# 87003697/DynamiCrafter

Measured on AMD Instinct MI355X. Metric: frames/sec (and denoising-step ms), 16f@576x1024, DDIM 50, higher is better.
Workload: dtype bf16; 1 GPU; inference_1024_v1.0.yaml: 1 clip/GPU, 16 frames, latent 72x128, DDIM 50 uniform_trailing eta=1, CFG 7.5 batched (cond+uncond), guidance_rescale 0.7, v-param+ZTSNR+dynamic rescale, hipGraph-captured step; clips_per_gpu=1, parallelism=dp1 over 1 distinct clips (no data-path collective), conditioning=local (1 rank), outputs_finite=True

## Files before the change

### dynamicrafter_amd/_hip.py

```python
import ctypes as C
import os
import threading

_HERE = os.path.dirname(os.path.abspath(__file__))
LIB_PATH = os.environ.get("DC_HIP_LIB") or os.path.join(_HERE, "csrc", "libdcrafter_hip.so")

DC_GEMM_OUT_F32 = 1
DC_GEMM_GEGLU = 2
DC_GEMM_GELU = 4


class DcGemmParams(C.Structure):
    _fields_ = [
        ("A", C.c_void_p), ("W", C.c_void_p), ("C", C.c_void_p), ("bias", C.c_void_p),
        ("rowvec", C.c_void_p), ("residual", C.c_void_p),
        ("lda", C.c_int), ("ldc", C.c_int), ("ldr", C.c_int), ("rowvec_ld", C.c_int),
        ("rows_per_vec", C.c_int),
        ("M", C.c_int), ("N", C.c_int), ("K", C.c_int), ("n_pad", C.c_int),
        ("mode", C.c_int), ("Cin", C.c_int),
        ("IH", C.c_int), ("IW", C.c_int), ("OH", C.c_int), ("OW", C.c_int),
        ("stride", C.c_int), ("pad", C.c_int), ("ups", C.c_int),
        ("T", C.c_int), ("HW", C.c_int),
        ("flags", C.c_int), ("alpha", C.c_float),
        ("workspace", C.c_void_p), ("workspace_bytes", C.c_longlong),
    ]


class DcDdimParams(C.Structure):
    _fields_ = [
        ("a_t", C.c_void_p), ("a_prev", C.c_void_p), ("sigma_t", C.c_void_p), ("sqrt_one_minus_at", C.c_void_p),
        ("sqrt_acp_t", C.c_void_p), ("sqrt_1macp_t", C.c_void_p), ("scale_ratio", C.c_void_p),
        ("step_index", C.c_void_p),
        ("index", C.c_int), ("v_param", C.c_int),
        ("cfg_scale", C.c_float), ("cfg_img", C.c_float), ("guidance_rescale", C.c_float),
        ("temperature", C.c_float),
        ("e_nchw", C.c_int), ("noise_step_stride", C.c_int64),
    ]


class DcDpmParams(C.Structure):
    _fields_ = [
        ("A", C.c_void_p), ("alpha_t", C.c_void_p), ("alpha_p_r", C.c_void_p), ("k", C.c_void_p), ("N", C.c_void_p),
        ("sqrt_one_minus_at", C.c_void_p), ("sqrt_acp_t", C.c_void_p), ("sqrt_1macp_t", C.c_void_p),
        ("scale_ratio", C.c_void_p), ("step_index", C.c_void_p),
        ("index", C.c_int), ("v_param", C.c_int),
        ("cfg_scale", C.c_float), ("cfg_img", C.c_float), ("guidance_rescale", C.c_float),
        ("temperature", C.c_float),
        ("e_nchw", C.c_int), ("noise_step_stride", C.c_int64), ("x0_hist", C.c_void_p),
    ]


class DcSdsParams(C.Structure):
    _fields_ = [
        ("c1", C.c_void_p), ("c2", C.c_void_p), ("w", C.c_void_p), ("step_size", C.c_void_p), ("bc2_sqrt", C.c_void_p),
        ("step_index", C.c_void_p), ("index", C.c_int), ("weight_type", C.c_int), ("x0_param", C.c_int),
        ("e_nchw", C.c_int), ("cfg_scale", C.c_float), ("guidance_rescale", C.c_float),
        ("beta2", C.c_float), ("eps", C.c_float), ("one_minus_beta1", C.c_float), ("one_minus_beta2", C.c_float),
        ("decay", C.c_float), ("grad_scale", C.c_float), ("noise_step_stride", C.c_int64), ("loss", C.c_void_p),
    ]


_P, _I, _F, _L = C.c_void_p, C.c_int, C.c_float, C.c_int64
SIGNATURES = {
    "dc_gemm_conv": (_I, [C.POINTER(DcGemmParams), _P]),
    "dc_gemm_workspace_bytes": (_L, []),
    "dc_gemm_last_variant": (C.c_char_p, []),
    "dc_gemm_set_plan": (_I, [_I]),
    "dc_groupnorm": (_I, [_P, _I, _P, _I, _P, _P, _I, _I, _I, _I, _F, _I, _P, _P]),
    "dc_groupnorm_workspace_bytes": (_L, [_I, _I, _I]),
    "dc_layernorm": (_I, [_P, _I, _P, _I, _P, _P, _I, _I, _F, _P]),
    "dc_flash_attn_d64": (_I, [_P, _P, _P, _P, _I, _I, _I, _I, _I, _I, _I, _I, _L, _L, _F, _I, _F, _P]),
    "dc_ff_geglu_fused320": (_I, [_P, _I, _P, _P, _F, _P, _P, _P, _P, _P, _I, _P, _I, _I, _P]),
    "dc_ff_geglu_proj_fused320": (_I, [_P, _I, _P, _P, _F, _P, _P, _P, _P, _P, _P, _P, _I, _P, _I, _I, _P]),
    "dc_ln_linear": (_I, [_P, _I, _I, _P, _P, _F, _P, _P, _P, _I, _I, _I, _P]),
    "dc_ln_qkv_temporal_attn320": (_I, [_P, _I, _P, _P, _F, _P, _P, _I, _I, _I, _I, _F, _P]),
    "dc_ln_qkv_temporal_attn640": (_I, [_P, _I, _P, _P, _F, _P, _P, _I, _I, _I, _I, _F, _P]),
    "dc_gn_silu_tconv3": (_I, [_P, _I, _I, _P, _P, _P, _I, _P, _P, _P, _I, _P, _I, _I, _I, _I, _I, _P]),
    "dc_groupnorm_stats": (_I, [_P, _I, _I, _I, _I, _I, _F, _P, _P, _P]),
    "dc_gn_linear": (_I, [_P, _I, _I, _P, _P, _P, _I, _I, _P, _P, _P, _I, _I, _I, _P]),
    "dc_flash_attn_set_mode": (_I, [_I, _F]),
    "dc_linear_residual": (_I, [_P, _I, _I, _P, _P, _P, _I, _P, _I, _I, _I, _P]),
    "dc_cross_attn_dual_d64": (_I, [_P, _P, _P, _P, _P, _P, _I, _I, _I, _I, _I, _I, _I, _I, _L, _L, _F, _F, _P]),
    "dc_temporal_attn_d64": (_I, [_P, _I, _P, _I, _I, _I, _I, _I, _F, _P]),
    "dc_gemv_small": (_I, [_P, _I, _P, _P, _P, _I, _I, _I, _I, _I, _I, _I, _P]),
    "dc_timestep_embedding": (_I, [_P, _P, _I, _P, _I, _I, _F, _P]),
    "dc_pack_latent": (_I, [_P, _P, _P, _I, _I, _I, _I, _I, _I, _I, _P]),
    "dc_pack_latent_windows": (_I, [_P, _P, _P, _P, _P] + [_I] * 13 + [_P]),
    "dc_window_merge": (_I, [_P, _I, _P, _I, _P, _P, _P] + [_I] * 12 + [_P]),
    "dc_nchw_to_rows": (_I, [_P, _P, _I, _I, _I, _I, _F, _P]),
    "dc_rows_to_nchw": (_I, [_P, _I, _I, _P, _I, _I, _I, _F, _P]),
    "dc_im2col3x3_c8": (_I, [_P, _I, _P, _I, _I, _I, _I, _P]),
    "dc_copy2d": (_I, [_P, _I, _P, _I, _I, _I, _P]),
    "dc_build_context": (_I, [_P, _P, _I, _I, _I, _I, _I, _P]),
    "dc_softmax_rows": (_I, [_P, _I, _P, _I, _I, _I, _P]),
    "dc_transpose": (_I, [_P, _I, _P, _I, _I, _I, _P]),
    "dc_add_rows": (_I, [_P, _I, _P, _I, _P, _I, _I, _I, _P]),
    "dc_vae_sample": (_I, [_P, _I, _P, _P, _I, _I, _I, _F, _P]),
    "dc_ddim_step": (_I, [C.POINTER(DcDdimParams), _P, _P, _P, _I, _P, _P, _P, _P, _I, _I, _I, _P, _P]),
    "dc_dpmpp_step": (_I, [C.POINTER(DcDpmParams), _P, _P, _P, _I, _P, _P, _P, _P, _I, _I, _I, _P, _P]),
    "dc_sds_noise": (_I, [C.POINTER(DcSdsParams), _P, _P, _P, _I, _L, _P]),
    "dc_sds_step": (_I, [C.POINTER(DcSdsParams), _P, _P, _I, _P, _P, _P, _P, _I, _I, _I, _P, _P]),
    "dc_attn_small": (_I, [_P, _P, _P, _P, _I, _I, _I, _I, _I, _I, _I, _I, _I, _F, _I, _P]),
    "dc_attn_small_lds_bytes": (_L, [_I, _I]),
    "dc_clip_preprocess": (_I, [_P, _P, _P, _P, _I, _I, _I, _I, _I, _I, _I, C.POINTER(_F), C.POINTER(_F), _P]),
    "dc_patchify": (_I, [_P, _P, _I, _I, _I, _I, _I, _I, _P]),
    "dc_embed_tokens": (_I, [_P, _P, _P, _P, _I, _I, _I, _I, _P]),
    "dc_frames_to_u8": (_I, [_P, _P, _I, _I, _I, _I, _I, _P]),
    "dc_jpeg_dct_quant": (_I, [_P, _P, _P, _I, _I, _I, _P]),
    "dc_jpeg_entropy": (_I, [_P, _P, _P, _I, _I, _I, _I, _L, _P]),
    "dc_jpeg_pack": (_I, [_P, _P, _P, _P, _P, _I, _I, _L, _L, _P]),
    "dc_mask_blend": (_I, [_P, _P, _P, _P, _P, _P, _P, _I, _L, _L, _I, _P]),
    "dc_advance_counter": (_I, [_P, _P]),
    "dc_stream_create": (_I, [C.POINTER(_P)]),
    "dc_stream_destroy": (_I, [_P]),
    "dc_stream_sync": (_I, [_P]),
    "dc_graph_begin_capture": (_I, [_P]),
    "dc_graph_end_capture": (_I, [_P, C.POINTER(_P)]),
    "dc_graph_launch": (_I, [_P, _P]),
    "dc_graph_destroy": (_I, [_P]),
    "dc_event_create": (_I, [C.POINTER(_P)]),
    "dc_event_record": (_I, [_P, _P]),
    "dc_event_elapsed_ms": (_I, [_P, _P, C.POINTER(_F)]),
    "dc_event_destroy": (_I, [_P]),
    "dc_error_word_read": (_I, [C.POINTER(C.c_int), _I]),
    "dc_version": (C.c_char_p, []),
}

_lib = None
_lock = threading.Lock()


def lib():
    global _lib
    if _lib is not None:
        return _lib
    with _lock:
        if _lib is None:
            if not os.path.exists(LIB_PATH):
                raise RuntimeError(
                    f"{LIB_PATH} not found: build it with dynamicrafter_amd/csrc/build.sh "
                    "(or __graft_entry__.build()); the HIP extension is mandatory, there is no fallback")
            import torch
            l = C.CDLL(LIB_PATH)
            for name, (res, args) in SIGNATURES.items():
                fn = getattr(l, name)
                fn.restype = res
                fn.argtypes = args
            _lib = l
    return _lib


ERROR_WORD_BITS = {1: "gemm_pipe320x16_kernel: LDS counter wait timed out",
                   2: "flash_attn_d64_pipe_kernel: K/V ring counter wait timed out",
                   4: "gemm_pp_kernel: LDS counter wait timed out"}


def check_error_word(what="", reset=True):
    w = C.c_int(0)
    check(lib().dc_error_word_read(C.byref(w), 1 if reset else 0), "dc_error_word_read")
    if w.value:
        names = [v for k, v in ERROR_WORD_BITS.items() if w.value & k] or [f"unknown bits {w.value:#x}"]
        raise RuntimeError(f"HIP kernels reported a failed wait ({what or 'error word'} = {w.value:#x}): " + "; ".join(names)
                           + " - results since the last check are NOT valid")


def check(code, what):
    if code != 0:
        raise RuntimeError(f"{what} failed with code {code}"
                           + (" (DC_ERR_SHAPE)" if code == -1 else " (DC_ERR_ARG)" if code == -2 else " (hipError_t)"))
```

### dynamicrafter_amd/csrc/norms.hip

```cpp
#include "dc_common.h"
#include "dcrafter_hip.h"
#include <stdlib.h>

namespace {

struct GnGeom { int chunks; int rows_per_chunk; };

__host__ __device__ inline GnGeom gn_geom(int n_inst, int rows_per_inst) {
    int chunks = (2048 + n_inst - 1) / n_inst;
    int rpc = (rows_per_inst + chunks - 1) / chunks;
    if (rpc < 64) rpc = 64;
    GnGeom g;
    g.rows_per_chunk = rpc;
    g.chunks = (rows_per_inst + rpc - 1) / rpc;
    return g;
}

__global__ void gn_partial_kernel(const bf16_t* __restrict__ x, int ldx, int C, int groups, int rows_per_inst,
                                  int rows_per_chunk, int chunks, int vecs, int rpp, float2* __restrict__ partial) {
    extern __shared__ float sm[];
    const int inst = blockIdx.y, chunk = blockIdx.x;
    const int v = threadIdx.x % vecs;
    const int ro = threadIdx.x / vecs;
    const int r_begin = chunk * rows_per_chunk;
// ... 43 lines not shown
        for (int rr = 0; rr < rpp; ++rr) {
            const int first = r_begin + rr;
            const float nb = first < r_end ? (float)((r_end - first + rpp - 1) / rpp) : 0.f;
            if (nb == 0.f) continue;
            for (int c = 0; c < cpg; ++c) {
                const float mb = sm_s[rr * C + g * cpg + c], qb = sm_q[rr * C + g * cpg + c];
                const float nn = n + nb;
                const float w = nb * __builtin_amdgcn_rcpf(nn);
                const float delta = mb - mean;
                mean += delta * w;
                m2 += qb + delta * delta * (n * w);
                n = nn;
            }
        }
        partial[((size_t)inst * chunks + chunk) * groups + g] = make_float2(mean, m2);
    }
}

__global__ __launch_bounds__(64) void gn_finalize_kernel(const float2* __restrict__ partial, int chunks, int groups,
                                                         int rows_per_inst, int rows_per_chunk, int cpg, float eps,
                                                         float2* __restrict__ stats) {
    const int g = blockIdx.x, inst = blockIdx.y;
    float n = 0.f, mean = 0.f, m2 = 0.f;
    for (int c = threadIdx.x; c < chunks; c += 64) {
        const float2 p = partial[((size_t)inst * chunks + c) * groups + g];
        int rows = rows_per_inst - c * rows_per_chunk;
        if (rows > rows_per_chunk) rows = rows_per_chunk;
        const float nb = (float)rows * (float)cpg;
        const float nn = n + nb;
        const float w = nb * __builtin_amdgcn_rcpf(nn);
        const float delta = p.x - mean;
        mean += delta * w;
        m2 += p.y + delta * delta * (n * w);
        n = nn;
    }
#pragma unroll
    for (int o = 32; o > 0; o >>= 1) {
        const float nb = __shfl_xor(n, o, 64), mb = __shfl_xor(mean, o, 64), qb = __shfl_xor(m2, o, 64);
        const float nn = n + nb;
        if (nn > 0.f) {
            const float w = nb * __builtin_amdgcn_rcpf(nn);
            const float delta = mb - mean;
            mean += delta * w;
            m2 += qb + delta * delta * (n * w);
            n = nn;
        }
    }
    if (threadIdx.x == 0) {
        float var = m2 / n;
        if (var < 0.f) var = 0.f;
        stats[(size_t)inst * groups + g] = make_float2(mean, rsqrtf(var + eps));
    }
}

template <bool FIN>
__global__ void gn_apply_kernel(const bf16_t* __restrict__ x, int ldx, bf16_t* __restrict__ y, int ldy,
                                const float* __restrict__ gamma, const float* __restrict__ beta, int C, int groups,
                                int rows_per_inst, int rows_per_chunk, int vecs, int rpp, int silu,
                                const float2* __restrict__ stats, int chunks, float eps) {
    const int inst = blockIdx.y, chunk = blockIdx.x;
    __shared__ float2 st_s[64];
    if constexpr (FIN) {
        const int t = threadIdx.x, sub = t & 7;
        const int gpp = (int)blockDim.x >> 3;
        const float cpg = (float)(C / groups);
        for (int g0 = 0; g0 < groups; g0 += gpp) {
            const int g = g0 + (t >> 3);
            float n = 0.f, mean = 0.f, m2 = 0.f;
            if (g < groups) {
                for (int c = sub; c < chunks; c += 8) {
                    const float2 p = stats[((size_t)inst * chunks + c) * groups + g];
                    int rows = rows_per_inst - c * rows_per_chunk;
                    if (rows > rows_per_chunk) rows = rows_per_chunk;
                    const float nb = (float)rows * cpg;
                    const float nn = n + nb;
                    const float w = nb * __builtin_amdgcn_rcpf(nn);
                    const float delta = p.x - mean;
                    mean += delta * w;
                    m2 += p.y + delta * delta * (n * w);
                    n = nn;
                }
            }
#pragma unroll
            for (int o = 1; o < 8; o <<= 1) {
                const float nb = __shfl_xor(n, o, 64), mb = __shfl_xor(mean, o, 64), qb = __shfl_xor(m2, o, 64);
                const float nn = n + nb;
                if (nn > 0.f) {
                    const float lo_n = (sub & o) ? nb : n, lo_m = (sub & o) ? mb : mean, lo_q = (sub & o) ? qb : m2;
                    const float hi_n = (sub & o) ? n : nb, hi_m = (sub & o) ? mean : mb, hi_q = (sub & o) ? m2 : qb;
                    const float w = hi_n * __builtin_amdgcn_rcpf(nn);
                    const float delta = hi_m - lo_m;
                    mean = lo_m + delta * w;
                    m2 = lo_q + hi_q + delta * delta * (lo_n * w);
                    n = nn;
                }
            }
            if (g < groups && sub == 0) {
                float var = m2 / n;
                if (var < 0.f) var = 0.f;
                st_s[g] = make_float2(mean, rsqrtf(var + eps));
            }
        }
        __syncthreads();
    }
    const int v = threadIdx.x % vecs;
    const int ro = threadIdx.x / vecs;
    const int r_begin = chunk * rows_per_chunk;
    int r_end = r_begin + rows_per_chunk;
    if (r_end > rows_per_inst) r_end = rows_per_inst;
    const int cpg = C / groups;
    float sc[8], sh[8];
#pragma unroll
    for (int e = 0; e < 8; ++e) {
        const int c = v * 8 + e;
        const float2 st = FIN ? st_s[c / cpg] : stats[(size_t)inst * groups + c / cpg];
        const float g = gamma[c] * st.y;
        sc[e] = g;
        sh[e] = beta[c] - st.x * g;
    }
    const bf16_t* xb = x + (size_t)inst * rows_per_inst * ldx + v * 8;
    bf16_t* yb = y + (size_t)inst * rows_per_inst * ldy + v * 8;
    int r = r_begin + ro;
    for (; r + 7 * rpp < r_end; r += 8 * rpp) {
        uint4 raw[8];
#pragma unroll
        for (int u = 0; u < 8; ++u) raw[u] = *reinterpret_cast<const uint4*>(xb + (size_t)(r + u * rpp) * ldx);
#pragma unroll
        for (int u = 0; u < 8; ++u) {
            float f[8];
            unpack_bf8(raw[u], f);
#pragma unroll
            for (int e = 0; e < 8; ++e) {
                float t = f[e] * sc[e] + sh[e];
                if (silu) t = silu_f(t);
                f[e] = t;
            }
            *reinterpret_cast<uint4*>(yb + (size_t)(r + u * rpp) * ldy) = pack_bf8(f);
        }
    }
    for (; r < r_end; r += rpp) {
        const uint4 raw = *reinterpret_cast<const uint4*>(xb + (size_t)r * ldx);
        float f[8];
        unpack_bf8(raw, f);
#pragma unroll
        for (int e = 0; e < 8; ++e) {
            float t = f[e] * sc[e] + sh[e];
            if (silu) t = silu_f(t);
            f[e] = t;
        }
        *reinterpret_cast<uint4*>(yb + (size_t)r * ldy) = pack_bf8(f);
    }
}

template <int MAXV>
__global__ __launch_bounds__(256) void layernorm_kernel(const bf16_t* __restrict__ x, int ldx, bf16_t* __restrict__ y,
                                                        int ldy, const float* __restrict__ gamma,
                                                        const float* __restrict__ beta, int rows, int C, float eps) {
    const int lane = threadIdx.x & 63;
    const int wave = threadIdx.x >> 6;
    const int vecs = C >> 3;
    const float invC = 1.0f / (float)C;
    for (int row0 = (blockIdx.x * 4 + wave) * 2; row0 < rows; row0 += gridDim.x * 8) {
        float f[2][MAXV][8];
        float s[2] = {0.f, 0.f};
#pragma unroll
        for (int u = 0; u < 2; ++u) {
            const int row = row0 + u < rows ? row0 + u : rows - 1;
#pragma unroll
            for (int j = 0; j < MAXV; ++j) {
                const int v = lane + 64 * j;
                if (v < vecs) {
                    const uint4 raw = *reinterpret_cast<const uint4*>(x + (size_t)row * ldx + v * 8);
                    unpack_bf8(raw, f[u][j]);
#pragma unroll
                    for (int e = 0; e < 8; ++e) s[u] += f[u][j][e];
                }
            }
        }
#pragma unroll
        for (int u = 0; u < 2; ++u) {
            const int row = row0 + u;
            const float mean = wave_sum(s[u]) * invC;
            float q = 0.f;
#pragma unroll
            for (int j = 0; j < MAXV; ++j) {
                const int v = lane + 64 * j;
                if (v < vecs) {
#pragma unroll
                    for (int e = 0; e < 8; ++e) { const float d = f[u][j][e] - mean; q += d * d; }
                }
            }
            const float rstd = rsqrtf(wave_sum(q) * invC + eps);
            if (row < rows) {
#pragma unroll
                for (int j = 0; j < MAXV; ++j) {
                    const int v = lane + 64 * j;
                    if (v < vecs) {
                        float o[8];
#pragma unroll
                        for (int e = 0; e < 8; ++e) {
                            const int c = v * 8 + e;
                            o[e] = (f[u][j][e] - mean) * rstd * gamma[c] + beta[c];
                        }
                        *reinterpret_cast<uint4*>(y + (size_t)row * ldy + v * 8) = pack_bf8(o);
                    }
                }
            }
        }
    }
}

}

extern "C" int64_t dc_groupnorm_workspace_bytes(int n_inst, int groups, int rows_per_inst) {
    const GnGeom g = gn_geom(n_inst, rows_per_inst);
    return (int64_t)sizeof(float2) * ((int64_t)n_inst * g.chunks * groups + (int64_t)n_inst * groups) + 256;
}

extern "C" int dc_groupnorm(const uint16_t* x, int ldx, uint16_t* y, int ldy, const float* gamma, const float* beta,
                            int C, int groups, int n_inst, int rows_per_inst, float eps, int silu,
                            float* workspace, void* stream_) {
    hipStream_t stream = (hipStream_t)stream_;
    if (!x || !y || !gamma || !beta || !workspace) return DC_ERR_ARG;
    if (C % 8 != 0 || groups <= 0 || groups > 64 || C % groups != 0 || ldx % 8 != 0 || ldy % 8 != 0) return DC_ERR_SHAPE;
    if (n_inst <= 0 || rows_per_inst <= 0) return DC_ERR_SHAPE;
    const int vecs = C / 8;
    if (vecs > 1024) return DC_ERR_SHAPE;
    int rpp = 256 / vecs;
    if (rpp < 1) rpp = 1;
    const int threads = vecs * rpp;
    const GnGeom g = gn_geom(n_inst, rows_per_inst);
    float2* partial = reinterpret_cast<float2*>(workspace);
    float2* stats = partial + (size_t)n_inst * g.chunks * groups;
    const size_t lds = (size_t)2 * rpp * C * sizeof(float);
    if (lds > 64 * 1024) return DC_ERR_SHAPE;
    hipLaunchKernelGGL(gn_partial_kernel, dim3(g.chunks, n_inst), dim3(threads), lds, stream, x, ldx, C, groups,
                       rows_per_inst, g.rows_per_chunk, g.chunks, vecs, rpp, partial);
    DC_CHECK_LAUNCH();
    static const bool fuse_fin = [] { const char* e = getenv("DC_GN_FUSE_FINALIZE"); return !(e && e[0] == '0'); }();
    if (fuse_fin && g.chunks <= 64 && threads % 8 == 0) {
        hipLaunchKernelGGL(gn_apply_kernel<true>, dim3(g.chunks, n_inst), dim3(threads), 0, stream, x, ldx, y, ldy, gamma, beta,
                           C, groups, rows_per_inst, g.rows_per_chunk, vecs, rpp, silu, (const float2*)partial, g.chunks, eps);
        DC_CHECK_LAUNCH();
        return 0;
    }
    hipLaunchKernelGGL(gn_finalize_kernel, dim3(groups, n_inst), dim3(64), 0, stream, partial, g.chunks, groups, rows_per_inst,
                       g.rows_per_chunk, C / groups, eps, stats);
    DC_CHECK_LAUNCH();
    hipLaunchKernelGGL(gn_apply_kernel<false>, dim3(g.chunks, n_inst), dim3(threads), 0, stream, x, ldx, y, ldy, gamma, beta,
                       C, groups, rows_per_inst, g.rows_per_chunk, vecs, rpp, silu, (const float2*)stats, g.chunks, eps);
    DC_CHECK_LAUNCH();
    return 0;
}

extern "C" int dc_groupnorm_stats(const uint16_t* x, int ldx, int C, int groups, int n_inst, int rows_per_inst, float eps,
                                  float* workspace, float* stats_out, void* stream_) {
    hipStream_t stream = (hipStream_t)stream_;
    if (!x || !workspace || !stats_out) return DC_ERR_ARG;
    if (C % 8 != 0 || groups <= 0 || groups > 64 || C % groups != 0 || ldx % 8 != 0) return DC_ERR_SHAPE;
    if (n_inst <= 0 || rows_per_inst <= 0) return DC_ERR_SHAPE;
    const int vecs = C / 8;
    if (vecs > 1024) return DC_ERR_SHAPE;
    int rpp = 256 / vecs;
    if (rpp < 1) rpp = 1;
    const int threads = vecs * rpp;
    const GnGeom g = gn_geom(n_inst, rows_per_inst);
    float2* partial = reinterpret_cast<float2*>(workspace);
    const size_t lds = (size_t)2 * rpp * C * sizeof(float);
    if (lds > 64 * 1024) return DC_ERR_SHAPE;
    hipLaunchKernelGGL(gn_partial_kernel, dim3(g.chunks, n_inst), dim3(threads), lds, stream, x, ldx, C, groups,
                       rows_per_inst, g.rows_per_chunk, g.chunks, vecs, rpp, partial);
    DC_CHECK_LAUNCH();
    hipLaunchKernelGGL(gn_finalize_kernel, dim3(groups, n_inst), dim3(64), 0, stream, partial, g.chunks, groups, rows_per_inst,
                       g.rows_per_chunk, C / groups, eps, reinterpret_cast<float2*>(stats_out));
    DC_CHECK_LAUNCH();
    return 0;
}

extern "C" int dc_layernorm(const uint16_t* x, int ldx, uint16_t* y, int ldy, const float* gamma, const float* beta,
                            int rows, int C, float eps, void* stream_) {
    hipStream_t stream = (hipStream_t)stream_;
    if (!x || !y || !gamma || !beta) return DC_ERR_ARG;
    if (C % 8 != 0 || C > 2048 || ldx % 8 != 0 || ldy % 8 != 0 || rows <= 0) return DC_ERR_SHAPE;
    int grid = (rows + 7) / 8;
    if (grid > 8192) grid = 8192;
    const int vecs = C / 8;
    if (vecs <= 64)
        hipLaunchKernelGGL(layernorm_kernel<1>, dim3(grid), dim3(256), 0, stream, x, ldx, y, ldy, gamma, beta, rows, C, eps);
    else if (vecs <= 128)
        hipLaunchKernelGGL(layernorm_kernel<2>, dim3(grid), dim3(256), 0, stream, x, ldx, y, ldy, gamma, beta, rows, C, eps);
    else
        hipLaunchKernelGGL(layernorm_kernel<4>, dim3(grid), dim3(256), 0, stream, x, ldx, y, ldy, gamma, beta, rows, C, eps);
    DC_CHECK_LAUNCH();
    return 0;
}
```

### dynamicrafter_amd/ops.py

```python
import ctypes as C
import os
import math

import torch

from . import _hip
from ._hip import DcDdimParams, DcGemmParams, check

_BF16 = torch.bfloat16


def stream_ptr():
    return C.c_void_p(torch.cuda.current_stream().cuda_stream)


class Tracer:

    def __init__(self):
        self.records = []

    def __enter__(self):
        global _TRACE
        _TRACE = self
        return self
# ... 138 lines not shown
    p.residual = 0 if residual is None else _rows(residual, "residual").data_ptr()
    p.ldr = 0 if residual is None else residual.stride(0)
    p.lda, p.ldc = a.stride(0), out.stride(0)
    p.M = out.shape[0] if M is None else M
    p.N, p.K, p.n_pad = pw.N, pw.K, pw.n_pad
    p.Cin = pw.Cin
    p.flags = (_hip.DC_GEMM_OUT_F32 if out_f32 else 0) | (_hip.DC_GEMM_GEGLU if geglu else 0) | \
        (_hip.DC_GEMM_GELU if gelu else 0)
    p.alpha = alpha
    ws = _gemm_workspace(a.device, torch.cuda.current_stream().cuda_stream)
    p.workspace, p.workspace_bytes = ws.data_ptr(), ws.numel()
    if conv is not None:
        p.mode = 1
        p.IH, p.IW, p.OH, p.OW = conv["IH"], conv["IW"], conv["OH"], conv["OW"]
        p.stride, p.pad, p.ups = conv.get("stride", 1), conv.get("pad", 1), conv.get("ups", 0)
        if pw.taps != 9 or a.shape[1] < pw.Cin:
            raise ValueError("conv3x3 weight / activation mismatch")
    elif tconv is not None:
        p.mode = 2
        p.T, p.HW = tconv["T"], tconv["HW"]
        if pw.taps != 3:
            raise ValueError("tconv weight mismatch")
    else:
        p.mode = 0
        if a.shape[1] < pw.K:
            raise ValueError(f"gemm: activation has {a.shape[1]} columns, weight K={pw.K}")
    n_out = pw.N // 2 if geglu else pw.N
    if out.shape[1] < n_out:
        raise ValueError(f"gemm: out has {out.shape[1]} columns, need {n_out}")
    if out.shape[0] < p.M or (residual is not None and (residual.shape[0] < p.M or residual.shape[1] < n_out)):
        raise ValueError(f"gemm: out/residual have fewer than M={p.M} rows (or residual fewer than {n_out} columns)")
    if p.mode == 1:
        if p.M % (p.OH * p.OW) != 0 or a.shape[0] < (p.M // (p.OH * p.OW)) * p.IH * p.IW:
            raise ValueError(f"conv3x3: M={p.M} output rows need {p.M // (p.OH * p.OW)} frames of {p.IH}x{p.IW} input rows, "
                             f"activation has {a.shape[0]}")
    elif a.shape[0] < p.M:
        raise ValueError(f"gemm: activation has {a.shape[0]} rows, M={p.M}")
    if p.mode == 2 and (p.M % (p.T * p.HW) != 0 or a.shape[1] < pw.Cin):
        raise ValueError("tconv: M must be a multiple of T*HW and the activation at least Cin wide")
    if rowvec is not None and (rowvec.shape[0] * rows_per_vec < p.M or rowvec.shape[1] < n_out):
        raise ValueError("gemm: rowvec does not cover every row group / output column")
    if _TRACE is not None:
        variant = "dc_gemm_conv"
        k_real = pw.k_real if pw.k_real else pw.K
        flops = 2.0 * p.M * pw.N * k_real
        esz = 4 if out_f32 else 2
        nbytes = 2.0 * p.M * (k_real if p.mode == 0 else pw.Cin) + 2.0 * pw.N * pw.K + esz * p.M * n_out \
            + (2.0 * p.M * n_out if residual is not None else 0)
        _launch(variant, flops, nbytes, _hip.lib().dc_gemm_conv, C.byref(p), stream_ptr(),
                tag=(p.mode, p.M, pw.N, k_real))
    else:
        check(_hip.lib().dc_gemm_conv(C.byref(p), stream_ptr()), "dc_gemm_conv")
    return out


_gemm_ws = {}


def _gemm_workspace(device, stream):
    key = (device.index, stream)
    buf = _gemm_ws.get(key)
    if buf is None:
        buf = torch.empty(int(_hip.lib().dc_gemm_workspace_bytes()), dtype=torch.uint8, device=device)
        _gemm_ws[key] = buf
    return buf


class Arena:
    GUARD = 8

    def __init__(self):
        self._bufs = {}
        self._guarded = {}
        self.guard = os.environ.get("DC_ARENA_GUARD", "0") == "1"

    def get(self, tag, rows, cols, dtype=_BF16, device=None, zero=False):
        key = (tag, rows, cols, dtype)
        b = self._bufs.get(key)
        if b is None:
            if rows * cols >= 2 ** 31:
                raise ValueError(f"scratch buffer {tag} [{rows} x {cols}] has 2^31 elements or more")
            if self.guard:
                G = self.GUARD
                whole = torch.empty((rows + 2 * G, cols), dtype=dtype, device=device)
                whole.fill_(self._sentinel(dtype))
                b = whole[G:G + rows]
                if zero:
                    b.zero_()
                self._guarded[key] = whole
            else:
                b = (torch.zeros if zero else torch.empty)((rows, cols), dtype=dtype, device=device)
            self._bufs[key] = b
        return b

    @staticmethod
    def _sentinel(dtype):
        return 12345.0 if dtype.is_floating_point else 0x5a

    def check(self):
        bad = []
        for (tag, rows, cols, dtype), whole in self._guarded.items():
            G = self.GUARD
            ref = torch.full((1,), self._sentinel(dtype), dtype=dtype, device=whole.device)
            if not (bool((whole[:G] == ref).all()) and bool((whole[G + rows:] == ref).all())):
                bad.append(f"{tag}[{rows}x{cols} {dtype}]")
        if bad:
            raise RuntimeError("scratch buffers overrun: " + ", ".join(bad))
        return len(self._guarded)

    def nbytes(self):
        return sum(b.numel() * b.element_size() for b in self._bufs.values())


_gn_ws = {}


_gn_ws_retired = []


def _gn_workspace(device, nbytes):
    key = (device.index, torch.cuda.current_stream().cuda_stream)
    buf = _gn_ws.get(key)
    if buf is None or buf.numel() * 4 < nbytes:
        if buf is not None:
            _gn_ws_retired.append(buf)
        buf = torch.empty((max(nbytes, 4 << 20) + 3) // 4, dtype=torch.float32, device=device)
        _gn_ws[key] = buf
    return buf


def _need(t, n, name):
    if t is not None and t.numel() < n:
        raise ValueError(f"{name}: {t.numel()} elements, the launch reads/writes {n}")


def _need_rows(t, rows, cols, name):
    if t.shape[0] < rows or t.shape[1] < cols:
        raise ValueError(f"{name}: shape {tuple(t.shape)}, the launch addresses [{rows}, {cols}]")


def groupnorm(x, y, gamma, beta, *, groups, n_inst, rows_per_inst, eps, silu):
    _rows(x, "x"); _rows(y, "y")
    _need_rows(x, n_inst * rows_per_inst, gamma.numel(), "x"); _need_rows(y, n_inst * rows_per_inst, gamma.numel(), "y")
    _need(beta, gamma.numel(), "beta")
    Cc = gamma.numel()
    l = _hip.lib()
    ws = _gn_workspace(x.device, int(l.dc_groupnorm_workspace_bytes(n_inst, groups, rows_per_inst)))
    _launch("groupnorm(2-3 kernels)", 0.0, 6.0 * n_inst * rows_per_inst * Cc, l.dc_groupnorm, _ptr(x), x.stride(0), _ptr(y),
            y.stride(0), _ptr(gamma), _ptr(beta), Cc, groups, n_inst, rows_per_inst, eps, 1 if silu else 0, _ptr(ws),
            stream_ptr())
    return y


def layernorm(x, y, gamma, beta, eps=1e-5):
    _rows(x, "x"); _rows(y, "y")
    _need_rows(x, x.shape[0], gamma.numel(), "x"); _need_rows(y, x.shape[0], gamma.numel(), "y"); _need(beta, gamma.numel(), "beta")
    _launch("layernorm", 0.0, 4.0 * x.shape[0] * gamma.numel(), _hip.lib().dc_layernorm, _ptr(x), x.stride(0), _ptr(y),
            y.stride(0), _ptr(gamma), _ptr(beta), x.shape[0], gamma.numel(), eps, stream_ptr())
    return y


def flash_attn(q, k, v, o, *, batch, heads, Lq, Lk, scale, accumulate=False, acc_scale=1.0, q_bstride=None,
               kv_bstride=None):
    for t, n in ((q, "q"), (k, "k"), (v, "v"), (o, "o")):
        _rows(t, n)
    qb = Lq if q_bstride is None else q_bstride
    kb = Lk if kv_bstride is None else kv_bstride
    _need_rows(q, (batch - 1) * qb + Lq, heads * 64, "q"); _need_rows(o, (batch - 1) * qb + Lq, heads * 64, "o")
    _need_rows(k, (batch - 1) * kb + Lk, heads * 64, "k"); _need_rows(v, (batch - 1) * kb + Lk, heads * 64, "v")
    _launch("flash_attn_d64(self)" if Lk > 128 else "flash_attn_d64(cross)", 4.0 * batch * heads * Lq * Lk * 64,
            2.0 * batch * heads * 64 * (2 * Lq + 2 * Lk), _hip.lib().dc_flash_attn_d64, _ptr(q), _ptr(k), _ptr(v), _ptr(o),
            q.stride(0), k.stride(0), v.stride(0), o.stride(0), batch, heads, Lq, Lk,
            Lq if q_bstride is None else q_bstride, Lk if kv_bstride is None else kv_bstride, scale,
            1 if accumulate else 0, acc_scale, stream_ptr())
    return o


def cross_attn_dual(q, k, v, k2, v2, o, *, batch, heads, Lq, Lk, Lk2, scale, scale2, kv_bstride):
    for t, n in ((q, "q"), (k, "k"), (v, "v"), (k2, "k2"), (v2, "v2"), (o, "o")):
        _rows(t, n)
    if len({k.stride(0), v.stride(0), k2.stride(0), v2.stride(0)}) != 1:
        raise ValueError("cross_attn_dual: k, v, k2, v2 must share one row stride")
    _need_rows(q, batch * Lq, heads * 64, "q"); _need_rows(o, batch * Lq, heads * 64, "o")
    _need_rows(k, (batch - 1) * kv_bstride + Lk, heads * 64, "k"); _need_rows(v, (batch - 1) * kv_bstride + Lk, heads * 64, "v")
    _need_rows(k2, (batch - 1) * kv_bstride + Lk2, heads * 64, "k2"); _need_rows(v2, (batch - 1) * kv_bstride + Lk2, heads * 64, "v2")
    _launch("flash_attn_d64(cross)", 4.0 * batch * heads * Lq * (Lk + Lk2) * 64, 2.0 * batch * heads * 64 * (2 * Lq + 2 * (Lk + Lk2)),
            _hip.lib().dc_cross_attn_dual_d64, _ptr(q), _ptr(k), _ptr(v), _ptr(k2), _ptr(v2), _ptr(o), q.stride(0), k.stride(0),
            o.stride(0), batch, heads, Lq, Lk, Lk2, Lq, kv_bstride, scale, scale2, stream_ptr())
    return o


def temporal_attn(qkv, o, *, B, T, HW, heads, scale):
    _rows(qkv, "qkv"); _rows(o, "o")
    _need_rows(qkv, B * T * HW, 3 * heads * 64, "qkv"); _need_rows(o, B * T * HW, heads * 64, "o")
    _launch("temporal_attn_d64", 4.0 * B * HW * heads * T * T * 64, 2.0 * B * T * HW * heads * 64 * 4,
            _hip.lib().dc_temporal_attn_d64, _ptr(qkv), qkv.stride(0), _ptr(o), o.stride(0), B, T, HW, heads, scale,
            stream_ptr())
    return o


def ff2_permuted(weight, device):
    w = weight.detach()
    N, K = w.shape
    pos = torch.arange(32)
    s_, h_, e_ = pos // 16, (pos // 8) % 2, pos % 8
    chan = 8 * (2 * s_ + e_ // 4) + 4 * h_ + e_ % 4
    idx = (torch.arange(K // 32)[:, None] * 32 + chan[None, :]).reshape(-1)
    n_pad = (N + 127) // 128 * 128
    out = torch.zeros((n_pad, K), dtype=_BF16, device=device)
    out[:N] = w[:, idx].to(device=device, dtype=_BF16)
    return out


def ff_geglu_fused320(x, pw1, w2p, b2, out, residual=None, ln=None, ln_eps=1e-5):
    _rows(x, "x"); _rows(out, "out")
    M = x.shape[0]
    if pw1.K != 320 or pw1.N != 2560 or pw1.bias is None or tuple(w2p.shape[1:]) != (1280,) or w2p.shape[0] < 320:
        raise ValueError("ff_geglu_fused320: dim must be 320 (ff1 [2560, 320] with bias, ff2 [320, 1280])")
    _need_rows(x, M, 320, "x"); _need_rows(out, M, 320, "out")
    if residual is not None:
        _rows(residual, "residual"); _need_rows(residual, M, 320, "residual")
    if ln is not None:
        _need(ln[0], 320, "ln gamma"); _need(ln[1], 320, "ln beta")
    flops = 2.0 * M * (2560 + 1280) * 320
    nbytes = 2.0 * M * 320 * (3 if residual is not None else 2) + 2.0 * (2560 * 320 + 320 * 1280)
    _launch("ff_geglu_fused320", flops, nbytes, _hip.lib().dc_ff_geglu_fused320, _ptr(x), x.stride(0),
            _ptr(None if ln is None else ln[0]), _ptr(None if ln is None else ln[1]), ln_eps, _ptr(pw1.w), _ptr(pw1.bias),
            _ptr(w2p), _ptr(b2), _ptr(residual), 0 if residual is None else residual.stride(0), _ptr(out), out.stride(0), M,
            stream_ptr())
    return out


def ff_geglu_proj_fused320(x, pw1, w2p, b2, wp, bp, residual2, out, ln=None, ln_eps=1e-5):
    _rows(x, "x"); _rows(out, "out"); _rows(residual2, "residual2")
    M = x.shape[0]
    if pw1.K != 320 or pw1.N != 2560 or pw1.bias is None or tuple(w2p.shape[1:]) != (1280,) or w2p.shape[0] < 320 \
            or tuple(wp.shape[1:]) != (320,) or wp.shape[0] < 320:
        raise ValueError("ff_geglu_proj_fused320: dim must be 320 (ff1 [2560, 320] with bias, ff2 [320, 1280], proj [320, 320])")
    if x.data_ptr() == out.data_ptr():
        raise ValueError("ff_geglu_proj_fused320: out must not alias x")
    _need_rows(x, M, 320, "x"); _need_rows(out, M, 320, "out"); _need_rows(residual2, M, 320, "residual2")
    _need(b2, 320, "b2"); _need(bp, 320, "bp")
    if ln is not None:
        _need(ln[0], 320, "ln gamma"); _need(ln[1], 320, "ln beta")
    _launch("ff_geglu_proj_fused320", 2.0 * M * (2560 + 1280 + 320) * 320, 2.0 * M * 320 * 3 + 2.0 * (2560 * 320 + 320 * 1280 + 320 * 320),
            _hip.lib().dc_ff_geglu_proj_fused320, _ptr(x), x.stride(0), _ptr(None if ln is None else ln[0]),
            _ptr(None if ln is None else ln[1]), ln_eps, _ptr(pw1.w), _ptr(pw1.bias), _ptr(w2p), _ptr(b2), _ptr(wp), _ptr(bp),
            _ptr(residual2), residual2.stride(0), _ptr(out), out.stride(0), M, stream_ptr())
    return out


def ln_linear(x, pw, out, ln=None, ln_eps=1e-5):
    _rows(x, "x"); _rows(out, "out")
    M, K = x.shape[0], pw.K
    if K not in (320, 640) or pw.N % 32:
        raise ValueError("ln_linear: K must be 320 or 640 and N a multiple of 32")
    _need_rows(x, M, K, "x"); _need_rows(out, M, pw.N, "out")
    if ln is not None:
        _need(ln[0], K, "ln gamma"); _need(ln[1], K, "ln beta")
    _launch("ln_linear", 2.0 * M * pw.N * K, 2.0 * M * (K + pw.N) + 2.0 * pw.N * K, _hip.lib().dc_ln_linear,
            _ptr(x), x.stride(0), K, _ptr(None if ln is None else ln[0]), _ptr(None if ln is None else ln[1]), ln_eps,
            _ptr(pw.w), _ptr(pw.bias), _ptr(out), out.stride(0), M, pw.N, stream_ptr())
    return out


def linear_residual(x, pw, residual, out):
    _rows(x, "x"); _rows(out, "out"); _rows(residual, "residual")
    M, K = x.shape[0], pw.K
    if K not in (320, 640) or pw.N % 32:
        raise ValueError("linear_residual: K must be 320 or 640 and N a multiple of 32")
    _need_rows(x, M, K, "x"); _need_rows(out, M, pw.N, "out"); _need_rows(residual, M, pw.N, "residual")
    _launch("linear_residual", 2.0 * M * pw.N * K, 2.0 * M * (K + 2 * pw.N) + 2.0 * pw.N * K, _hip.lib().dc_linear_residual,
            _ptr(x), x.stride(0), K, _ptr(pw.w), _ptr(pw.bias), _ptr(residual), residual.stride(0), _ptr(out), out.stride(0),
            M, pw.N, stream_ptr())
    return out


def ln_qkv_temporal_attn(x, ln, pw_qkv, out, *, B, T, HW, scale, ln_eps=1e-5):
    _rows(x, "x"); _rows(out, "out")
    M = B * T * HW
    Cc = pw_qkv.K
    if Cc not in (320, 640) or pw_qkv.N != 3 * Cc or pw_qkv.bias is not None or T != 16 or HW % 8:
        raise ValueError("ln_qkv_temporal_attn: dim 320 / 640 (qkv weight [3 C, C], no bias), T = 16, HW % 8 == 0")
    if x.data_ptr() == out.data_ptr():
        raise ValueError("ln_qkv_temporal_attn: out must not alias x")
    _need_rows(x, M, Cc, "x"); _need_rows(out, M, Cc, "out"); _need(ln[0], Cc, "ln gamma"); _need(ln[1], Cc, "ln beta")
    fn = _hip.lib().dc_ln_qkv_temporal_attn320 if Cc == 320 else _hip.lib().dc_ln_qkv_temporal_attn640
    _launch(f"ln_qkv_temporal_attn{Cc}", 2.0 * M * 3 * Cc * Cc + 4.0 * M * T * Cc, 4.0 * M * Cc + 2.0 * 3 * Cc * Cc,
            fn, _ptr(x), x.stride(0), _ptr(ln[0]), _ptr(ln[1]), ln_eps, _ptr(pw_qkv.w),
            _ptr(out), out.stride(0), B, T, HW, scale, stream_ptr())
    return out


def ln_qkv_temporal_attn320(x, ln, pw_qkv, out, *, B, T, HW, scale, ln_eps=1e-5):
    if pw_qkv.K != 320:
        raise ValueError("ln_qkv_temporal_attn320: dim 320 (qkv weight [960, 320], no bias), T = 16, HW % 8 == 0")
    return ln_qkv_temporal_attn(x, ln, pw_qkv, out, B=B, T=T, HW=HW, scale=scale, ln_eps=ln_eps)


def gn_silu_tconv3(x, gamma, beta, stats, pw, out, *, B, T, HW, groups=32, residual=None):
    _rows(x, "x"); _rows(out, "out")
    M = B * T * HW
    C = pw.w.shape[1] // 3
    if C not in (320, 640) or pw.w.shape[1] != 3 * C or pw.N % 32 or pw.bias is None or T != 16 or HW % 8:
        raise ValueError("gn_silu_tconv3: 320 / 640 input channels (weight [N, 3 C] with bias), N % 32 == 0, T = 16, HW % 8 == 0")
    if x.data_ptr() == out.data_ptr():
# ... 467 lines not shown
```

### include/dcrafter_hip.h

```cpp
#ifndef DCRAFTER_HIP_H
#define DCRAFTER_HIP_H
#include <stdint.h>

#ifdef __cplusplus
extern "C" {
#endif

#define DC_ERR_SHAPE (-1)
#define DC_ERR_ARG   (-2)

#define DC_GEMM_OUT_F32 1
#define DC_GEMM_GEGLU   2
#define DC_GEMM_GELU    4

typedef struct DcGemmParams {
    const uint16_t* A;
    const uint16_t* W;
    void* C;
    const float* bias;
    const float* rowvec;
    const uint16_t* residual;
    int lda, ldc, ldr, rowvec_ld;
    int rows_per_vec;
    int M, N, K, n_pad;
    int mode;
    int Cin;
    int IH, IW, OH, OW;
    int stride, pad, ups;
    int T, HW;
    int flags;
    float alpha;
    void* workspace;
    long long workspace_bytes;
} DcGemmParams;

const char* dc_gemm_last_variant(void);

int dc_gemm_set_plan(int plan);

int64_t dc_gemm_workspace_bytes(void);

int dc_gemm_conv(const DcGemmParams* p, void* stream);

int dc_groupnorm(const uint16_t* x, int ldx, uint16_t* y, int ldy, const float* gamma, const float* beta,
                 int C, int groups, int n_inst, int rows_per_inst, float eps, int silu,
                 float* workspace, void* stream);
int64_t dc_groupnorm_workspace_bytes(int n_inst, int groups, int rows_per_inst);

int dc_layernorm(const uint16_t* x, int ldx, uint16_t* y, int ldy, const float* gamma, const float* beta,
                 int rows, int C, float eps, void* stream);

int dc_flash_attn_d64(const uint16_t* q, const uint16_t* k, const uint16_t* v, uint16_t* o,
                      int ldq, int ldk, int ldv, int ldo, int batch, int heads, int Lq, int Lk,
                      int64_t q_bstride, int64_t kv_bstride, float scale, int accumulate, float acc_scale,
                      void* stream);

int dc_flash_attn_set_mode(int mode, float thr);

int dc_temporal_attn_d64(const uint16_t* qkv, int ld, uint16_t* o, int ldo, int B, int T, int HW, int heads,
                         float scale, void* stream);

int dc_gemv_small(const float* in, int ld_in, const uint16_t* W, const float* bias, float* out, int ld_out,
                  int M, int N, int K, int act_in, int act_out, int accumulate, void* stream);

int dc_timestep_embedding(const int64_t* t_table, const int32_t* t_index, int t_stride, float* out, int B, int dim,
                          float max_period, void* stream);

int dc_pack_latent(const float* x, const float* cc, uint16_t* out, int B, int Cx, int Cc, int T, int HW,
                   int c_pad, int nrep, void* stream);

int dc_pack_latent_windows(const float* x, const float* cc, uint16_t* out, const int32_t* starts,
                           const int32_t* step_index, int index, int S, int W, int w0, int n_w, int B, int Cx, int Cc,
                           int T_long, int T, int HW, int c_pad, int nrep, void* stream);

int dc_window_merge(const float* e, int ld_e, float* out, int ld_out, const int32_t* starts, const float* wn,
                    const int32_t* step_index, int index, int S, int W, int w0, int n_w, int nb, int B, int C, int T_long,
                    int T, int HW, int accumulate, void* stream);

int dc_nchw_to_rows(const float* x, uint16_t* out, int N, int C, int HW, int c_pad, float scale, void* stream);
int dc_rows_to_nchw(const void* rows, int ld, int rows_f32, float* y, int N, int C, int HW, float scale, void* stream);

int dc_im2col3x3_c8(const uint16_t* x, int ldx, uint16_t* out, int ldo, int n_img, int H, int W, void* stream);

int dc_copy2d(const uint16_t* src, int lds, uint16_t* dst, int ldd, int rows, int cols, void* stream);

int dc_build_context(const float* ctx, uint16_t* out, int B, int T, int n_text, int L, int D, void* stream);

int dc_softmax_rows(const float* x, int ldx, uint16_t* y, int ldy, int rows, int cols, void* stream);

int dc_transpose(const uint16_t* src, int lds, uint16_t* dst, int ldd, int rows, int cols, void* stream);

int dc_add_rows(const uint16_t* a, int lda, const uint16_t* b, int ldb, uint16_t* y, int ldy, int rows, int cols,
                void* stream);

int dc_vae_sample(const uint16_t* moments, int ld, const float* noise, float* z, int N, int zc, int HW,
                  float scale, void* stream);

typedef struct DcDdimParams {
    const float* a_t;
    const float* a_prev;
    const float* sigma_t;
    const float* sqrt_one_minus_at;
    const float* sqrt_acp_t;
    const float* sqrt_1macp_t;
    const float* scale_ratio;
    const int32_t* step_index;
    int index;
    int v_param;
    float cfg_scale;
    float cfg_img;
    float guidance_rescale;
    float temperature;
    int e_nchw;
    int64_t noise_step_stride;
} DcDdimParams;

int dc_ddim_step(const DcDdimParams* p, const float* e_cond, const float* e_uncond, const float* e_img, int ld_e,
                 const float* x, const float* noise, float* x_prev, float* pred_x0, int B, int C, int THW,
                 float* workspace, void* stream);

typedef struct DcDpmParams {
    const float* A;
    const float* alpha_t;
    const float* alpha_p_r;
    const float* k;
    const float* N;
    const float* sqrt_one_minus_at;
    const float* sqrt_acp_t;
    const float* sqrt_1macp_t;
    const float* scale_ratio;
    const int32_t* step_index;
    int index;
    int v_param;
    float cfg_scale;
    float cfg_img;
    float guidance_rescale;
    float temperature;
    int e_nchw;
    int64_t noise_step_stride;
    float* x0_hist;
} DcDpmParams;

int dc_dpmpp_step(const DcDpmParams* p, const float* e_cond, const float* e_uncond, const float* e_img, int ld_e,
                  const float* x, const float* noise, float* x_prev, float* pred_x0, int B, int C, int THW,
                  float* workspace, void* stream);

typedef struct DcSdsParams {
    const float* c1;
    const float* c2;
    const float* w;
    const float* step_size;
    const float* bc2_sqrt;
    const int32_t* step_index;
    int index;
    int weight_type;
    int x0_param;
    int e_nchw;
    float cfg_scale;
    float guidance_rescale;
    float beta2, eps;
    float one_minus_beta1;
    float one_minus_beta2;
    float decay;
    float grad_scale;
    int64_t noise_step_stride;
    float* loss;
} DcSdsParams;

int dc_sds_noise(const DcSdsParams* p, const float* latent, const float* noise, float* x_t, int B, int64_t n_per_clip,
                 void* stream);

int dc_sds_step(const DcSdsParams* p, const float* e_cond, const float* e_uncond, int ld_e, const float* x_t,
                float* latent, float* m, float* v, int B, int C, int THW, float* workspace, void* stream);

int dc_cross_attn_dual_d64(const uint16_t* q, const uint16_t* k, const uint16_t* v, const uint16_t* k2, const uint16_t* v2,
                           uint16_t* o, int ldq, int ldkv, int ldo, int batch, int heads, int Lq, int Lk, int Lk2,
                           int64_t q_bstride, int64_t kv_bstride, float scale, float scale2, void* stream);

int dc_ff_geglu_fused320(const uint16_t* x, int ldx, const float* ln_gamma, const float* ln_beta, float ln_eps,
                         const uint16_t* w1, const float* b1, const uint16_t* w2p, const float* b2, const uint16_t* residual,
                         int ldr, uint16_t* out, int ldo, int M, void* stream);

int dc_ff_geglu_proj_fused320(const uint16_t* x, int ldx, const float* ln_gamma, const float* ln_beta, float ln_eps,
                              const uint16_t* w1, const float* b1, const uint16_t* w2p, const float* b2, const uint16_t* wp,
                              const float* bp, const uint16_t* residual2, int ldr2, uint16_t* out, int ldo, int M, void* stream);

int dc_ln_linear(const uint16_t* x, int ldx, int K, const float* ln_gamma, const float* ln_beta, float ln_eps, const uint16_t* w,
                 const float* bias, uint16_t* out, int ldo, int M, int N, void* stream);
int dc_groupnorm_stats(const uint16_t* x, int ldx, int C, int groups, int n_inst, int rows_per_inst, float eps,
                       float* workspace, float* stats_out, void* stream);
int dc_gn_linear(const uint16_t* x, int ldx, int K, const float* gamma, const float* beta, const float* stats, int groups,
                 int rows_per_inst, const uint16_t* w, const float* bias, uint16_t* out, int ldo, int M, int N, void* stream);

int dc_linear_residual(const uint16_t* x, int ldx, int K, const uint16_t* w, const float* bias, const uint16_t* residual, int ldr,
                       uint16_t* out, int ldo, int M, int N, void* stream);

int dc_ln_qkv_temporal_attn320(const uint16_t* x, int ldx, const float* ln_gamma, const float* ln_beta, float ln_eps,
                               const uint16_t* wqkv, uint16_t* out, int ldo, int B, int T, int HW, float scale, void* stream);
int dc_ln_qkv_temporal_attn640(const uint16_t* x, int ldx, const float* ln_gamma, const float* ln_beta, float ln_eps,
                               const uint16_t* wqkv, uint16_t* out, int ldo, int B, int T, int HW, float scale, void* stream);
// ... 58 lines not shown
```

Before: 2.664 frames/s.

## Add register-resident single-pass GroupNorm kernel for eligible shapes

Adds a GroupNorm kernel in which each block loads its slab of a group instance into registers once, computes the mean and then the centred variance with LDS reductions, and writes the normalized (optionally SiLU) output without re-reading global memory. It replaces the stats-then-apply multi-kernel path whenever a planner finds a thread and vector configuration that fits, and is on by default through an environment or API mode. The goal is to cut global memory traffic and the extra launch. The cost is heavy register pressure from up to 24 uint4 values per thread, plus lower parallelism when there are few instances and groups, which could hurt occupancy on large spatial shapes.

Result: no change. 2.681 frames/s (median of 6 runs) (+0.6%).

```diff
diff --git a/dynamicrafter_amd/_hip.py b/dynamicrafter_amd/_hip.py
--- a/dynamicrafter_amd/_hip.py
+++ b/dynamicrafter_amd/_hip.py
@@ -68,6 +68,8 @@
     "dc_gemm_set_plan": (_I, [_I]),
     "dc_groupnorm": (_I, [_P, _I, _P, _I, _P, _P, _I, _I, _I, _I, _F, _I, _P, _P]),
     "dc_groupnorm_workspace_bytes": (_L, [_I, _I, _I]),
+    "dc_groupnorm_set_onepass": (_I, [_I]),
+    "dc_groupnorm_onepass_eligible": (_I, [_I, _I, _I, _I]),
     "dc_layernorm": (_I, [_P, _I, _P, _I, _P, _P, _I, _I, _F, _P]),
     "dc_flash_attn_d64": (_I, [_P, _P, _P, _P, _I, _I, _I, _I, _I, _I, _I, _I, _L, _L, _F, _I, _F, _P]),
     "dc_ff_geglu_fused320": (_I, [_P, _I, _P, _P, _F, _P, _P, _P, _P, _P, _I, _P, _I, _I, _P]),
diff --git a/dynamicrafter_amd/csrc/norms.hip b/dynamicrafter_amd/csrc/norms.hip
--- a/dynamicrafter_amd/csrc/norms.hip
+++ b/dynamicrafter_amd/csrc/norms.hip
@@ -219,6 +219,200 @@
     }
 }
 
+#define GN1_NV_SMALL 24
+#define GN1_NV_BIG 13
+
+__device__ __forceinline__ void gn1_fold(const float* ch, float* part, int W, int cpg, int g, int rpp, int nwaves, int wpg) {
+    const int wave = threadIdx.x >> 6, lane = threadIdx.x & 63;
+    const int nterms = rpp * cpg;
+    for (int u = wave; u < g * wpg; u += nwaves) {
+        const int G = u / wpg, p = u - G * wpg;
+        float a = 0.f;
+        for (int i = p * 64 + lane; i < nterms; i += 64 * wpg) {
+            const int r = i / cpg, c = i - r * cpg;
+            a += ch[r * W + G * cpg + c];
+        }
+        a = wave_sum(a);
+        if (lane == 0) part[u] = a;
+    }
+}
+
+template <int T, int NV>
+__global__ __launch_bounds__(T) void gn_onepass_kernel(const bf16_t* __restrict__ x, int ldx, bf16_t* __restrict__ y, int ldy,
+                                                       const float* __restrict__ gamma, const float* __restrict__ beta,
+                                                       int cpg, int g, int spi, int rows, int vpr, int rpp, int silu,
+                                                       float eps) {
+    __shared__ float ch_s[T * 8];
+    __shared__ float part_s[64];
+    __shared__ float mean_s[64];
+    __shared__ float rstd_s[64];
+    const int L = xcd_remap(blockIdx.x, gridDim.x);
+    const int inst = L / spi, slab = L - inst * spi;
+    const int tid = threadIdx.x;
+    const bool active = tid < vpr * rpp;
+    const int ro = active ? tid / vpr : 0;
+    const int col = active ? tid - ro * vpr : 0;
+    const int n_t = active && ro < rows ? (rows - ro + rpp - 1) / rpp : 0;
+    const int c0 = slab * g * cpg + col * 8;
+    const char* xb = reinterpret_cast<const char*>(x + (size_t)inst * rows * ldx + slab * g * cpg);
+    uint4 raw[NV];
+#pragma unroll
+    for (int j = 0; j < NV; ++j) {
+        int r = ro + j * rpp;
+        if (r > rows - 1) r = rows - 1;
+        raw[j] = *reinterpret_cast<const uint4*>(xb + (uint32_t)(r * ldx + col * 8) * 2u);
+    }
+    float sc[8], sh[8];
+#pragma unroll
+    for (int e = 0; e < 8; ++e) { sc[e] = gamma[c0 + e]; sh[e] = beta[c0 + e]; }
+    const int ge0 = (col * 8) / cpg;
+    uint32_t gd = 0;
+    {
+        int gi = 0, rem = col * 8 - ge0 * cpg;
+#pragma unroll
+        for (int e = 0; e < 8; ++e) {
+            gd |= (uint32_t)gi << (2 * e);
+            if (++rem == cpg) { rem = 0; ++gi; }
+        }
+    }
+#define GN1_GE(e) (ge0 + (int)((gd >> (2 * (e))) & 3u))
+#define GN1_KEEP_RAW() _Pragma("unroll") for (int j = 0; j < NV; ++j) \
+        asm volatile("" : "+v"(raw[j].x), "+v"(raw[j].y), "+v"(raw[j].z), "+v"(raw[j].w))
+    const int W = vpr * 8;
+    const int nwaves = T / 64;
+    const int wpg = g < nwaves ? nwaves / g : 1;
+    const float inv_n = 1.0f / ((float)rows * (float)cpg);
+    float s[8];
+#pragma unroll
+    for (int e = 0; e < 8; ++e) s[e] = 0.f;
+#pragma unroll
+    for (int j = 0; j < NV; ++j) {
+        if (j < n_t) {
+            float f[8];
+            unpack_bf8(raw[j], f);
+#pragma unroll
+            for (int e = 0; e < 8; ++e) s[e] += f[e];
+        }
+    }
+    if (active) {
+#pragma unroll
+        for (int e = 0; e < 8; ++e) ch_s[tid * 8 + e] = s[e];
+    }
+    __syncthreads();
+    gn1_fold(ch_s, part_s, W, cpg, g, rpp, nwaves, wpg);
+    __syncthreads();
+    if (tid < g) {
+        float a = 0.f;
+        for (int p = 0; p < wpg; ++p) a += part_s[tid * wpg + p];
+        mean_s[tid] = a * inv_n;
+    }
+    __syncthreads();
+    float m[8];
+#pragma unroll
+    for (int e = 0; e < 8; ++e) m[e] = mean_s[GN1_GE(e)];
+    GN1_KEEP_RAW();
+#pragma unroll
+    for (int e = 0; e < 8; ++e) s[e] = 0.f;
+#pragma unroll
+    for (int j = 0; j < NV; ++j) {
+        if (j < n_t) {
+            float f[8];
+            unpack_bf8(raw[j], f);
+#pragma unroll
+            for (int e = 0; e < 8; ++e) { const float d = f[e] - m[e]; s[e] += d * d; }
+        }
+    }
+    if (active) {
+#pragma unroll
+        for (int e = 0; e < 8; ++e) ch_s[tid * 8 + e] = s[e];
+    }
+    __syncthreads();
+    gn1_fold(ch_s, part_s, W, cpg, g, rpp, nwaves, wpg);
+    __syncthreads();
+    if (tid < g) {
+        float a = 0.f;
+        for (int p = 0; p < wpg; ++p) a += part_s[tid * wpg + p];
+        rstd_s[tid] = rsqrtf(a * inv_n + eps);
+    }
+    __syncthreads();
+#pragma unroll
+    for (int e = 0; e < 8; ++e) {
+        const float gm = sc[e] * rstd_s[GN1_GE(e)];
+        sc[e] = gm;
+        sh[e] = sh[e] - m[e] * gm;
+    }
+    char* yb = reinterpret_cast<char*>(y + (size_t)inst * rows * ldy + slab * g * cpg);
+    GN1_KEEP_RAW();
+#pragma unroll
+    for (int j = 0; j < NV; ++j) {
+        if (j < n_t) {
+            float f[8];
+            unpack_bf8(raw[j], f);
+#pragma unroll
+            for (int e = 0; e < 8; ++e) {
+                float t = f[e] * sc[e] + sh[e];
+                if (silu) t = silu_f(t);
+                f[e] = t;
+            }
+            *reinterpret_cast<uint4*>(yb + (uint32_t)((ro + j * rpp) * ldy + col * 8) * 2u) = pack_bf8(f);
+        }
+    }
+}
+
+#undef GN1_KEEP_RAW
+#undef GN1_GE
+
+struct Gn1Plan { int g, threads, nv, vpr, rpp; };
+
+inline bool gn1_fits(int threads, int nv_max, int vpr, int rows, Gn1Plan* p) {
+    if (vpr > threads) return false;
+    const int rpp = threads / vpr;
+    const int nv = (rows + rpp - 1) / rpp;
+    if (nv > nv_max) return false;
+    p->threads = threads; p->nv = nv; p->vpr = vpr; p->rpp = rpp;
+    return true;
+}
+
+inline bool gn1_plan(int C, int groups, int n_inst, int rows, int ldmax, int mode, Gn1Plan* p) {
+    if ((int64_t)rows * ldmax * 2 >= (int64_t)1 << 31) return false;
+    if (mode <= 0 || C % 8 != 0 || groups <= 0 || groups > 64 || C % groups != 0 || n_inst <= 0 || rows <= 0) return false;
+    const int cpg = C / groups;
+    bool found = false;
+    for (int g = 1; g <= groups && !found; ++g) {
+        if (groups % g != 0 || (g * cpg) % 64 != 0) continue;
+        if (gn1_fits(256, GN1_NV_SMALL, g * cpg / 8, rows, p)) { p->g = g; found = true; }
+    }
+    for (int pass = 0; pass < 2 && !found; ++pass)
+        for (int g = groups; g >= 1 && !found; --g) {
+            if (groups % g != 0 || (g * cpg) % 8 != 0) continue;
+            if (gn1_fits(pass ? 1024 : 256, pass ? GN1_NV_BIG : GN1_NV_SMALL, g * cpg / 8, rows, p)) { p->g = g; found = true; }
+        }
+    if (!found) return false;
+    if (mode == 1 && p->threads == 1024 && p->g * cpg * 2 < 128 && (int64_t)n_inst * (groups / p->g) >= 256) return false;
+    return true;
+}
+
+std::atomic<int> gn1_mode{-1};
+
+inline int gn1_mode_now() {
+    int m = gn1_mode.load(std::memory_order_relaxed);
+    if (m < 0) {
+        const char* e = getenv("DC_GN_ONEPASS");
+        m = (e && e[0] >= '0' && e[0] <= '2' && e[1] == 0) ? e[0] - '0' : 1;
+        int expect = -1;
+        if (!gn1_mode.compare_exchange_strong(expect, m)) m = expect;
+    }
+    return m;
+}
+
+template <int T, int NV>
+inline void gn1_launch(const Gn1Plan& pl, const bf16_t* x, int ldx, bf16_t* y, int ldy, const float* gamma, const float* beta,
+                       int cpg, int groups, int n_inst, int rows, int silu, float eps, hipStream_t stream) {
+    const int spi = groups / pl.g;
+    hipLaunchKernelGGL((gn_onepass_kernel<T, NV>), dim3(n_inst * spi), dim3(T), 0, stream, x, ldx, y, ldy, gamma, beta, cpg, pl.g,
+                       spi, rows, pl.vpr, pl.rpp, silu, eps);
+}
+
 template <int MAXV>
 __global__ __launch_bounds__(256) void layernorm_kernel(const bf16_t* __restrict__ x, int ldx, bf16_t* __restrict__ y,
                                                         int ldy, const float* __restrict__ gamma,
@@ -293,6 +487,22 @@
     if (n_inst <= 0 || rows_per_inst <= 0) return DC_ERR_SHAPE;
     const int vecs = C / 8;
     if (vecs > 1024) return DC_ERR_SHAPE;
+    Gn1Plan pl;
+    if (gn1_plan(C, groups, n_inst, rows_per_inst, ldx > ldy ? ldx : ldy, gn1_mode_now(), &pl)) {
+#define GN1_CASE(T, NV) gn1_launch<T, NV>(pl, x, ldx, y, ldy, gamma, beta, C / groups, groups, n_inst, rows_per_inst, silu, eps, stream)
+        if (pl.threads == 256) {
+            if (pl.nv <= 4) GN1_CASE(256, 4);
+            else if (pl.nv <= 8) GN1_CASE(256, 8);
+            else if (pl.nv <= 16) GN1_CASE(256, 16);
+            else GN1_CASE(256, GN1_NV_SMALL);
+        } else {
+            if (pl.nv <= 7) GN1_CASE(1024, 7);
+            else GN1_CASE(1024, GN1_NV_BIG);
+        }
+#undef GN1_CASE
+        DC_CHECK_LAUNCH();
+        return 0;
+    }
     int rpp = 256 / vecs;
     if (rpp < 1) rpp = 1;
     const int threads = vecs * rpp;
@@ -318,6 +528,18 @@
                        C, groups, rows_per_inst, g.rows_per_chunk, vecs, rpp, silu, (const float2*)stats, g.chunks, eps);
     DC_CHECK_LAUNCH();
     return 0;
+}
+
+extern "C" int dc_groupnorm_set_onepass(int mode) {
+    if (mode < 0 || mode > 2) return DC_ERR_ARG;
+    const int prev = gn1_mode_now();
+    gn1_mode.store(mode, std::memory_order_relaxed);
+    return prev;
+}
+
+extern "C" int dc_groupnorm_onepass_eligible(int C, int groups, int n_inst, int rows_per_inst) {
+    Gn1Plan pl;
+    return gn1_plan(C, groups, n_inst, rows_per_inst, C, 1, &pl) ? pl.threads : 0;
 }
 
 extern "C" int dc_groupnorm_stats(const uint16_t* x, int ldx, int C, int groups, int n_inst, int rows_per_inst, float eps,
diff --git a/dynamicrafter_amd/ops.py b/dynamicrafter_amd/ops.py
--- a/dynamicrafter_amd/ops.py
+++ b/dynamicrafter_amd/ops.py
@@ -314,6 +314,17 @@
     return y
 
 
+def groupnorm_set_onepass(mode):
+    prev = _hip.lib().dc_groupnorm_set_onepass(int(mode))
+    if prev < 0:
+        raise ValueError(f"groupnorm_set_onepass: mode {mode}")
+    return prev
+
+
+def groupnorm_onepass_eligible(C, groups, n_inst, rows_per_inst):
+    return int(_hip.lib().dc_groupnorm_onepass_eligible(C, groups, n_inst, rows_per_inst))
+
+
 def layernorm(x, y, gamma, beta, eps=1e-5):
     _rows(x, "x"); _rows(y, "y")
     _need_rows(x, x.shape[0], gamma.numel(), "x"); _need_rows(y, x.shape[0], gamma.numel(), "y"); _need(beta, gamma.numel(), "beta")
diff --git a/include/dcrafter_hip.h b/include/dcrafter_hip.h
--- a/include/dcrafter_hip.h
+++ b/include/dcrafter_hip.h
@@ -46,6 +46,9 @@
                  int C, int groups, int n_inst, int rows_per_inst, float eps, int silu,
                  float* workspace, void* stream);
 int64_t dc_groupnorm_workspace_bytes(int n_inst, int groups, int rows_per_inst);
+
+int dc_groupnorm_set_onepass(int mode);
+int dc_groupnorm_onepass_eligible(int C, int groups, int n_inst, int rows_per_inst);
 
 int dc_layernorm(const uint16_t* x, int ldx, uint16_t* y, int ldy, const float* gamma, const float* beta,
                  int rows, int C, float eps, void* stream);
```
